# kan-bayashi/ParallelWaveGAN

Measured on AMD Instinct MI355X. Metric: HiFi-GAN V1 22.05 kHz generator inference RTF^-1 (audio samples/s), higher is better.
Workload: dtype f32; 1 GPU; HiFi-GAN V1 generator fwd, LJSpeech 22.05 kHz, B16 x 800 mel frames per GPU, fp32, random init; global_batch=16, parallelism=replicas x1

## Files before the change

### include/pwg_kernels.h

```cpp
#ifndef PWG_KERNELS_H_
#define PWG_KERNELS_H_

#include <stddef.h>
#include <stdint.h>

#ifdef __cplusplus
extern "C" {
#endif

typedef enum pwg_status {
  PWG_OK = 0,
  PWG_ERR_BAD_SHAPE = -1,
  PWG_ERR_UNSUPPORTED = -2,
  PWG_ERR_LAUNCH = -3,
  PWG_ERR_NULL = -4,
  PWG_ERR_WORKSPACE = -5
} pwg_status;

const char* pwg_last_error(void);
int pwg_abi_version(void);
int pwg_target_arch(void);

int pwg_prof_enable(int on);
int pwg_prof_reset(void);
// ... 64 lines not shown
int pwg_conv1d_backward_weight(const pwg_conv1d_desc* d, const float* x, const float* dy, float* dw,
                               float* db, float* workspace, size_t workspace_floats, void* stream);

size_t pwg_conv1d_backward_weight_wn_workspace_floats(const pwg_conv1d_desc* d);
int pwg_conv1d_backward_weight_wn(const pwg_conv1d_desc* d, const float* x, const float* dy, const float* v,
                                  const float* g, float* dv, float* dg, float* db, float* workspace,
                                  size_t workspace_floats, void* stream);

int pwg_conv1d_num_tile_configs(void);
int pwg_conv1d_forward_cfg(const pwg_conv1d_desc* d, const float* x, const float* w_packed,
                           const float* bias, const float* add1, const float* add2, float* y,
                           int32_t tile_config, int32_t use_dma, void* stream);

int pwg_conv1d_bf16_supported(const pwg_conv1d_desc* d);
size_t pwg_conv1d_bf16_packed_weight_bytes(const pwg_conv1d_desc* d);
int pwg_conv1d_bf16_pack_weight(const pwg_conv1d_desc* d, const float* w, const float* scale, void* w_packed,
                                void* stream);
int pwg_conv1d_bf16_forward(const pwg_conv1d_desc* d, const float* x, const void* w_packed, const float* bias,
                            const float* add1, const float* add2, float* y, float* workspace, size_t workspace_floats,
                            void* stream);
int pwg_conv1d_bf16_forward_cfg(const pwg_conv1d_desc* d, const float* x, const void* w_packed, const float* bias,
                                const float* add1, const float* add2, float* y, int32_t mfma_shape, void* stream);

int pwg_conv1d_split_supported(const pwg_conv1d_desc* d);
size_t pwg_conv1d_split_packed_weight_bytes(const pwg_conv1d_desc* d);
int pwg_conv1d_split_pack_weight(const pwg_conv1d_desc* d, const float* w, const float* scale, void* w_packed,
                                 void* stream);
int pwg_conv1d_split_forward(const pwg_conv1d_desc* d, const float* x, const void* w_packed, const float* bias,
                             const float* add1, const float* add2, float* y, float* workspace, size_t workspace_floats,
                             void* stream);
int pwg_conv1d_split_forward_cfg(const pwg_conv1d_desc* d, const float* x, const void* w_packed, const float* bias,
                                 const float* add1, const float* add2, float* y, int32_t mfma_shape, int32_t tile_mode,
                                 void* stream);

int pwg_conv1d_stream_supported(const pwg_conv1d_desc* d);
size_t pwg_conv1d_stream_hist_floats(const pwg_conv1d_desc* d);
int pwg_conv1d_stream_forward(const pwg_conv1d_desc* d, const float* x, const float* hist_in, float* hist_out,
                              const float* w_packed, const float* bias, const float* add1, const float* add2, float* y,
                              void* stream);

int pwg_conv1d_stream_bf16_supported(const pwg_conv1d_desc* d);
int pwg_conv1d_stream_bf16_forward(const pwg_conv1d_desc* d, const float* x, const float* hist_in, float* hist_out,
                                   const void* w_packed_bf16, const float* bias, const float* add1,
                                   const float* add2, float* y, void* stream);

int pwg_conv1d_stream_delayed_supported(const pwg_conv1d_desc* d, int32_t delay1, int32_t delay2);
int pwg_conv1d_stream_delayed_forward(const pwg_conv1d_desc* d, const float* x, const float* hist_in, float* hist_out,
                                      const float* w_packed, const float* bias, const float* add1,
                                      const float* add1_hist_in, float* add1_hist_out, int32_t delay1, const float* add2,
                                      const float* add2_hist_in, float* add2_hist_out, int32_t delay2, int32_t valid_lo,
                                      int32_t valid_hi, float* y, void* stream);

int pwg_conv1d_stream_bf16_delayed_supported(const pwg_conv1d_desc* d, int32_t delay1, int32_t delay2);
int pwg_conv1d_stream_bf16_delayed_forward(const pwg_conv1d_desc* d, const float* x, const float* hist_in,
                                           float* hist_out, const void* w_packed_bf16, const float* bias,
                                           const float* add1, const float* add1_hist_in, float* add1_hist_out,
                                           int32_t delay1, const float* add2, const float* add2_hist_in,
                                           float* add2_hist_out, int32_t delay2, int32_t valid_lo, int32_t valid_hi,
                                           float* y, void* stream);

int pwg_conv1d_stream_mirrored_supported(const pwg_conv1d_desc* d);
int pwg_conv1d_stream_mirrored_forward(const pwg_conv1d_desc* d, const float* x, const float* hist_in, float* hist_out,
                                       const float* w_packed, const float* bias, float* y, int32_t in_lo, int32_t in_hi,
                                       int32_t valid_lo, int32_t valid_hi, void* stream);

int pwg_conv1d_plan(const pwg_conv1d_desc* d, int32_t has_addends, int32_t* out);
// ... 310 lines not shown
```

### parallelwavegan_amd/_lib.py

```python
import ctypes
import os

_HERE = os.path.dirname(os.path.abspath(__file__))
LIB_PATH = os.environ.get("PWG_KERNEL_LIB") or os.path.join(_HERE, "libpwgkernels.so")

PWG_ACT_NONE, PWG_ACT_LEAKY_RELU, PWG_ACT_TANH, PWG_ACT_RELU = 0, 1, 2, 3
PWG_PAD_ZERO, PWG_PAD_REFLECT, PWG_PAD_REPLICATE = 0, 1, 2
ABI_VERSION = 15
SPECTRAL_NORM_SCRATCH_FLOATS = 257


class ConvDesc(ctypes.Structure):

    _fields_ = [
        ("batch", ctypes.c_int32),
        ("c_in", ctypes.c_int32),
        ("c_out", ctypes.c_int32),
        ("t_in", ctypes.c_int32),
        ("t_out", ctypes.c_int32),
        ("width", ctypes.c_int32),
        ("kernel", ctypes.c_int32),
        ("stride", ctypes.c_int32),
        ("dilation", ctypes.c_int32),
        ("pad_left", ctypes.c_int32),
# ... 76 lines not shown
_i64 = ctypes.c_int64
_f32 = ctypes.c_float

SIGNATURES = {
    "pwg_last_error": (ctypes.c_char_p, []),
    "pwg_abi_version": (ctypes.c_int, []),
    "pwg_target_arch": (ctypes.c_int, []),
    "pwg_debug_poison_lds": (ctypes.c_int, [ctypes.c_int]),
    "pwg_set_concurrency_hint": (ctypes.c_float, [ctypes.c_float]),
    "pwg_prof_enable": (ctypes.c_int, [ctypes.c_int]),
    "pwg_prof_reset": (ctypes.c_int, []),
    "pwg_prof_num_kernels": (ctypes.c_int, []),
    "pwg_prof_get": (ctypes.c_int, [_i32, ctypes.c_char_p, ctypes.c_size_t, ctypes.POINTER(ctypes.c_double),
                                    ctypes.POINTER(ctypes.c_int64), ctypes.POINTER(ctypes.c_double),
                                    ctypes.POINTER(ctypes.c_double)]),
    "pwg_conv1d_packed_weight_floats": (ctypes.c_size_t, [ctypes.POINTER(ConvDesc)]),
    "pwg_conv1d_pack_weight": (ctypes.c_int, [ctypes.POINTER(ConvDesc), _vp, _vp, _vp, _vp]),
    "pwg_conv1d_forward_workspace_floats": (ctypes.c_size_t, [ctypes.POINTER(ConvDesc)]),
    "pwg_conv1d_forward": (ctypes.c_int, [ctypes.POINTER(ConvDesc), _vp, _vp, _vp, _vp, _vp, _vp, _vp, ctypes.c_size_t,
                                          _vp]),
    "pwg_conv1d_bf16_supported": (ctypes.c_int, [ctypes.POINTER(ConvDesc)]),
    "pwg_conv1d_bf16_packed_weight_bytes": (ctypes.c_size_t, [ctypes.POINTER(ConvDesc)]),
    "pwg_conv1d_bf16_pack_weight": (ctypes.c_int, [ctypes.POINTER(ConvDesc), _vp, _vp, _vp, _vp]),
    "pwg_conv1d_bf16_forward": (ctypes.c_int, [ctypes.POINTER(ConvDesc), _vp, _vp, _vp, _vp, _vp, _vp, _vp, ctypes.c_size_t,
                                               _vp]),
    "pwg_conv1d_bf16_forward_cfg": (ctypes.c_int, [ctypes.POINTER(ConvDesc), _vp, _vp, _vp, _vp, _vp, _vp, _i32, _vp]),
    "pwg_conv1d_split_supported": (ctypes.c_int, [ctypes.POINTER(ConvDesc)]),
    "pwg_conv1d_split_packed_weight_bytes": (ctypes.c_size_t, [ctypes.POINTER(ConvDesc)]),
    "pwg_conv1d_split_pack_weight": (ctypes.c_int, [ctypes.POINTER(ConvDesc), _vp, _vp, _vp, _vp]),
    "pwg_conv1d_split_forward": (ctypes.c_int, [ctypes.POINTER(ConvDesc), _vp, _vp, _vp, _vp, _vp, _vp, _vp,
                                                ctypes.c_size_t, _vp]),
    "pwg_conv1d_split_forward_cfg": (ctypes.c_int, [ctypes.POINTER(ConvDesc), _vp, _vp, _vp, _vp, _vp, _vp, _i32, _i32,
                                                    _vp]),
    "pwg_conv1d_stream_supported": (ctypes.c_int, [ctypes.POINTER(ConvDesc)]),
    "pwg_conv1d_stream_hist_floats": (ctypes.c_size_t, [ctypes.POINTER(ConvDesc)]),
    "pwg_conv1d_stream_forward": (ctypes.c_int, [ctypes.POINTER(ConvDesc), _vp, _vp, _vp, _vp, _vp, _vp, _vp, _vp, _vp]),
    "pwg_conv1d_stream_bf16_supported": (ctypes.c_int, [ctypes.POINTER(ConvDesc)]),
    "pwg_conv1d_stream_bf16_forward": (ctypes.c_int, [ctypes.POINTER(ConvDesc), _vp, _vp, _vp, _vp, _vp, _vp, _vp, _vp,
                                                      _vp]),
    "pwg_conv1d_stream_delayed_supported": (ctypes.c_int, [ctypes.POINTER(ConvDesc), _i32, _i32]),
    "pwg_conv1d_stream_delayed_forward": (ctypes.c_int, [ctypes.POINTER(ConvDesc), _vp, _vp, _vp, _vp, _vp, _vp, _vp, _vp,
                                                         _i32, _vp, _vp, _vp, _i32, _i32, _i32, _vp, _vp]),
    "pwg_conv1d_stream_bf16_delayed_supported": (ctypes.c_int, [ctypes.POINTER(ConvDesc), _i32, _i32]),
    "pwg_conv1d_stream_bf16_delayed_forward": (ctypes.c_int, [ctypes.POINTER(ConvDesc), _vp, _vp, _vp, _vp, _vp, _vp, _vp,
                                                              _vp, _i32, _vp, _vp, _vp, _i32, _i32, _i32, _vp, _vp]),
    "pwg_conv1d_stream_mirrored_supported": (ctypes.c_int, [ctypes.POINTER(ConvDesc)]),
    "pwg_conv1d_stream_mirrored_forward": (ctypes.c_int, [ctypes.POINTER(ConvDesc), _vp, _vp, _vp, _vp, _vp, _vp, _i32,
                                                          _i32, _i32, _i32, _vp]),
    "pwg_conv1d_packed_weight_bwd_floats": (ctypes.c_size_t, [ctypes.POINTER(ConvDesc)]),
    "pwg_conv1d_pack_weight_bwd": (ctypes.c_int, [ctypes.POINTER(ConvDesc), _vp, _vp, _vp, _vp]),
    "pwg_weight_bank_table_bytes": (ctypes.c_size_t, [_i32]),
    "pwg_weight_bank_build": (ctypes.c_int, [ctypes.POINTER(BankItem), _i32, _vp, ctypes.c_size_t,
                                             ctypes.POINTER(ctypes.c_int32)]),
    "pwg_weight_bank_prepare": (ctypes.c_int, [_vp, ctypes.POINTER(ctypes.c_int32), _i32, _vp]),
    "pwg_conv1d_backward_data_workspace_floats": (ctypes.c_size_t, [ctypes.POINTER(ConvDesc)]),
    "pwg_conv1d_backward_data": (ctypes.c_int, [ctypes.POINTER(ConvDesc), _vp, _vp, _vp, _vp, _vp, _vp, ctypes.c_size_t,
                                                _vp]),
    "pwg_conv1d_backward_weight_workspace_floats": (ctypes.c_size_t, [ctypes.POINTER(ConvDesc)]),
    "pwg_conv1d_backward_weight": (ctypes.c_int, [ctypes.POINTER(ConvDesc), _vp, _vp, _vp, _vp, _vp, ctypes.c_size_t, _vp]),
    "pwg_conv1d_backward_weight_wn_workspace_floats": (ctypes.c_size_t, [ctypes.POINTER(ConvDesc)]),
    "pwg_conv1d_backward_weight_wn": (ctypes.c_int, [ctypes.POINTER(ConvDesc), _vp, _vp, _vp, _vp, _vp, _vp, _vp, _vp,
                                                     ctypes.c_size_t, _vp]),
    "pwg_conv1d_num_tile_configs": (ctypes.c_int, []),
    "pwg_conv1d_forward_cfg": (ctypes.c_int, [ctypes.POINTER(ConvDesc), _vp, _vp, _vp, _vp, _vp, _vp, _i32, _i32, _vp]),
    "pwg_conv1d_plan": (ctypes.c_int, [ctypes.POINTER(ConvDesc), _i32, ctypes.POINTER(_i32)]),
    "pwg_conv1d_backward_weight_plan": (ctypes.c_int, [ctypes.POINTER(ConvDesc), _i32, _i32, ctypes.POINTER(_i32)]),
# ... 147 lines not shown
```

### parallelwavegan_amd/csrc/conv1d_split.hip

```cpp
#include "mfma_conv.h"

namespace pwg {
namespace {

constexpr int PARTS = 3;

struct SplitArgs : MfmaConvArgs {
  int plane;
  long part_stride;
  float pre_mul;
  unsigned pre_mask;
  int wide_out;
};

static int split_geometry(const pwg_conv1d_desc* d, MfmaConvGeom* g) {
  return mfma_conv_geometry("conv1d_split", PARTS, false, d, g);
}

__device__ __forceinline__ float pre_activate(float v, float mul, unsigned mask) {
  const float n = __uint_as_float(__float_as_uint(v * mul) & mask);
  return v > 0.f ? v : n;
}

template <int NT, bool CHECKED>
// ... 186 lines not shown
    }
    __syncthreads();
    for (int tap = 0; tap < a.taps; ++tap) {
#pragma unroll
      for (int ks = 0; ks < KSTEPS; ++ks) {
        const int oct = ks * HL + c.h;
        const bf16x8* __restrict__ wp =
            image_rows(a.w, a.cin_chunks, a.m_pad, tap, chunk, oct) + c.m0 + c.wave_m * (WM * 32) + c.r;
        split_step<TILE, TM, TN, kConvRow, true>(wp, a.part_stride, xs, c.sh + c.wave_n * (WN * 32) + c.r + tap * a.dil,
                                                 oct * 8, a.plane, acc);
      }
    }
  }

  const size_t out_base = (size_t)c.b * a.c_out * a.t_out;
  const int row0 = c.m0 + c.wave_m * (WM * 32) + c.r, col0 = c.q0 + c.wave_n * (WN * 32) + 4 * c.h;
  const bool full = c.m0 + MT <= a.m && c.q0 + NT <= a.nq;
  if (!a.wide_out)
    split_epilogue<TILE, TM, TN, false, false>(a, acc, row0, col0, out_base);
  else if (full)
    split_epilogue<TILE, TM, TN, true, true>(a, acc, row0, col0, out_base);
  else
    split_epilogue<TILE, TM, TN, true, false>(a, acc, row0, col0, out_base);
}

template <bool VEC>
struct Family {
  template <int TILE, int WM, int WN, int WAVES_M>
  struct K {
    static constexpr auto fn = conv1d_split_mfma_kernel<TILE, WM, WN, WAVES_M, VEC>;
  };
};

static int split_forward(const pwg_conv1d_desc* d, const float* x, const void* w_packed, const float* bias,
                         const float* add1, const float* add2, float* y, int mfma_shape, int tile_mode,
                         hipStream_t stream) {
  MfmaConvGeom g;
  int rc = split_geometry(d, &g);
  if (rc == PWG_OK) rc = mfma_conv_check_forward("conv1d_split", d, x, w_packed, y, mfma_shape, tile_mode);
  if (rc != PWG_OK) return rc;
  const MfmaConvPlan p = mfma_conv_plan(d, g, PARTS, tile_mode, x, add1, add2);
  SplitArgs a;
  mfma_conv_fill_args(&a, d, g, x, w_packed, bias, add1, add2, y);
  a.plane = p.plane;
  a.part_stride = image_elems(g) / 8;
  a.pre_mul = d->pre_act == PWG_ACT_LEAKY_RELU ? d->pre_slope : (d->pre_act == PWG_ACT_RELU ? 0.0f : 1.0f);
  a.pre_mask = d->pre_act == PWG_ACT_RELU ? 0u : ~0u;
  a.wide_out = d->t_out % 4 == 0 && ((reinterpret_cast<uintptr_t>(y) | reinterpret_cast<uintptr_t>(add1) |
                                      reinterpret_cast<uintptr_t>(add2)) & 15u) == 0;
  maybe_poison_lds(stream);
  ProfScope prof(stream, "conv1d_split_mfma_kernel", p.flops, p.bytes);
  if (p.vec)
    mfma_conv_launch<Family<true>::K>(p, mfma_shape, a, stream);
  else
    mfma_conv_launch<Family<false>::K>(p, mfma_shape, a, stream);
  PWG_CHECK_LAUNCH("conv1d_split");
  return PWG_OK;
}

constexpr int kDefaultMfmaShape = 16;

}
}

using namespace pwg;

extern "C" int pwg_conv1d_split_supported(const pwg_conv1d_desc* d) {
  MfmaConvGeom g;
  return split_geometry(d, &g) == PWG_OK ? 1 : 0;
}

extern "C" size_t pwg_conv1d_split_packed_weight_bytes(const pwg_conv1d_desc* d) {
  MfmaConvGeom g;
  if (split_geometry(d, &g) != PWG_OK) return 0;
  return (size_t)PARTS * image_elems(g) * sizeof(__bf16);
}

extern "C" int pwg_conv1d_split_pack_weight(const pwg_conv1d_desc* d, const float* w, const float* scale, void* w_packed,
                                            void* stream) {
  MfmaConvGeom g;
  int rc = split_geometry(d, &g);
  if (rc != PWG_OK) return rc;
  PWG_REQUIRE(w && w_packed, PWG_ERR_NULL, "conv1d_split_pack_weight: NULL pointer");
  mfma_conv_pack<PARTS>(d, g, w, scale, w_packed, (hipStream_t)stream);
  PWG_CHECK_LAUNCH("conv1d_split_pack_weight");
  return PWG_OK;
}

extern "C" int pwg_conv1d_split_forward(const pwg_conv1d_desc* d, const float* x, const void* w_packed, const float* bias,
                                        const float* add1, const float* add2, float* y, float* workspace,
                                        size_t workspace_floats, void* stream) {
  (void)workspace;
  (void)workspace_floats;
  return split_forward(d, x, w_packed, bias, add1, add2, y, kDefaultMfmaShape, 0, (hipStream_t)stream);
}

extern "C" int pwg_conv1d_split_forward_cfg(const pwg_conv1d_desc* d, const float* x, const void* w_packed,
                                            const float* bias, const float* add1, const float* add2, float* y,
                                            int32_t mfma_shape, int32_t tile_mode, void* stream) {
  return split_forward(d, x, w_packed, bias, add1, add2, y, mfma_shape, tile_mode, (hipStream_t)stream);
}
```

### parallelwavegan_amd/functional.py

```python
import ctypes
import math
import os

import torch

from . import _lib, ops
from .ops import _ptr, _require_device, _stream

_L = _lib.lib


def _c(t):
    return t if t.is_contiguous() else t.contiguous()


class WeightNormFn(torch.autograd.Function):

    @staticmethod
    def forward(ctx, v, g):
        v = _c(v)
        g = _c(g)
        scale = ops.weight_norm_scale(v, g.reshape(-1))
        ctx.save_for_backward(v, g)
        return ops.scale_rows(v, scale)
# ... 29 lines not shown
class SpectralNormFn(torch.autograd.Function):

    @staticmethod
    def forward(ctx, w_orig, u, v, do_iter, eps):
        w_orig = _c(w_orig)
        _require_device(w_orig, u, v)
        rows = w_orig.shape[0]
        cols = w_orig.numel() // rows
        sigma = torch.empty(1, device=w_orig.device, dtype=torch.float32)
        w = torch.empty_like(w_orig)
        tmp = torch.empty(max(rows, 32 * cols), device=w_orig.device, dtype=torch.float32)
        u_saved, v_saved = (torch.empty_like(u), torch.empty_like(v)) if do_iter else (u.clone(), v.clone())
        _lib.check(_L().pwg_spectral_norm_forward_saved(_ptr(w_orig), _ptr(u), _ptr(v), _ptr(sigma), _ptr(w), _ptr(tmp),
                                                        _ptr(u_saved), _ptr(v_saved), rows, cols, int(bool(do_iter)),
                                                        float(eps), _stream()), "spectral_norm_forward_saved")
        ctx.save_for_backward(w_orig, u_saved, v_saved, sigma)
        return w

    @staticmethod
    def backward(ctx, dw):
        w_orig, u, v, sigma = ctx.saved_tensors
        dw = _c(dw)
        rows = w_orig.shape[0]
        cols = w_orig.numel() // rows
        dwo = torch.empty_like(w_orig)
        scratch = torch.empty(_lib.SPECTRAL_NORM_SCRATCH_FLOATS, device=dw.device, dtype=torch.float32)
        _lib.check(_L().pwg_spectral_norm_backward(_ptr(dw), _ptr(w_orig), _ptr(u), _ptr(v), _ptr(sigma), _ptr(dwo),
                                                   _ptr(scratch), rows, cols, _stream()), "spectral_norm_backward")
        return dwo, None, None, None, None


class PreparedWeights:

    __slots__ = ("key", "w", "_scale", "_fwd", "_fwd_desc", "_bwd", "_res", "_bf16", "_split", "_stale")

    def __init__(self, key, w, scale, fwd=None, fwd_desc=None, bwd=None):
        self.key, self.w, self._scale, self._fwd, self._fwd_desc, self._bwd, self._res = key, w, scale, fwd, fwd_desc, bwd, None
        self._bf16 = None
        self._split = None
        self._stale = False

    @property
    def scale(self):
        self._check()
        return self._scale

    def _check(self):
        if self._stale:
            raise RuntimeError("these prepared weights were overwritten by a later WeightBank.ensure(): a backward pass "
                               "through a graph built before the last parameter update is not supported with a "
                               "weight bank (call backward before the optimizer step, or disable the bank)")

    def _image(self, slot, pack, *desc):
        self._check()
        img = getattr(self, slot)
        if img is None:
            with torch.no_grad():
                img = pack(*desc, self.w, self._scale)
            setattr(self, slot, img)
        return img

    @property
    def fwd(self):
        return self._image("_fwd", ops.pack_weight, self._fwd_desc)

    def res(self):
        return self._image("_res", ops.resunit_pack_weight)

    def bf16(self):
        return self._image("_bf16", ops.pack_weight_bf16, self._fwd_desc)

    def split(self):
        return self._image("_split", ops.pack_weight_split, self._fwd_desc)

    def bwd(self, desc):
        return self._image("_bwd", ops.pack_weight_bwd, desc)


class FusedConvFn(torch.autograd.Function):

    @staticmethod
    def forward(ctx, x, w, bias, add1, add2, geom, fused, packed, g=None, precomputed=None):
        x = _c(x)
        b = x.shape[0]
        width = geom.get("width", 1)
        t_in = x.shape[-1] // width if x.dim() == 3 else x.shape[2]
        x3 = x.reshape(b, x.shape[1], -1)
        c_in = x3.shape[1]
        transposed = geom["transposed"]
        k = geom["kernel"]
        if transposed:
            c_out = w.shape[1] * geom["groups"]
            t_out = ops.conv_transpose_out_length(t_in, k, geom["stride"], geom["padding"], geom["output_padding"])
        else:
            c_out = w.shape[0]
            t_out = geom.get("t_out")
            if t_out is None:
                t_out = ops.conv_out_length(t_in, k, geom["stride"], geom["dilation"], geom["padding"],
                                            geom.get("padding_right", geom["padding"]))
        desc = ops.make_conv_desc(b, c_in, c_out, t_in, t_out, k, geom["stride"], geom["dilation"], geom["padding"],
                                  geom["groups"], transposed=transposed, width=width,
                                  pad_mode=geom.get("pad_mode", "zero"), **fused)
        wc = _c(w.reshape(w.shape[0], w.shape[1], -1))
        holder = packed if isinstance(packed, PreparedWeights) else None
        if holder is None:
            scale = None
# ... 870 lines not shown
```

### parallelwavegan_amd/layers/conv.py

```python
import math
import os

import torch

from .. import functional as Fn
from .. import ops


class _ConvNd(torch.nn.Module):
    transposed = False
    width_mode = False
    explicit_pad_min_elems = 1 << 20
    fold_batch = {"0": False, "1": True}.get(os.environ.get("PWG_FOLD_BATCH", ""), True)
    fold_max_cols = int(os.environ.get("PWG_FOLD_MAX_COLS", 40))
    fold_min_weight_bytes = 4 << 20
    precision = "fp32"
    split_exact = {"0": False, "1": True}.get(os.environ.get("PWG_SPLIT_EXACT", ""), True)
    split_admit_all = False

    def __init__(self, in_channels, out_channels, kernel_size, stride=1, padding=0, dilation=1, groups=1,
                 bias=True, output_padding=0, pad_mode="zero"):
        super().__init__()
        if in_channels % groups or out_channels % groups:
            raise ValueError("in_channels and out_channels must be divisible by groups")
# ... 133 lines not shown
            with torch.no_grad():
                if self.has_weight_norm:
                    v = self._w3(self.weight_v.detach())
                    scale = ops.weight_norm_scale(v, self.weight_g.detach().reshape(-1).contiguous())
                    self._cache_packed = Fn.PreparedWeights(key, v, scale, None, desc)
                else:
                    w = self._w3(self.effective_weight())
                    self._cache_packed = Fn.PreparedWeights(key, w, None, None, desc)
        return self._cache_packed

    def adopt_prepared(self, pw):
        self._cache_packed = pw

    def holds_current(self, pw):
        return self._cache_packed is pw and pw.key == self._params_key()

    def _packed(self, pack, cached):
        if self.has_spectral_norm and self.training:
            return pack(self.make_desc(1, self._probe_len()), self._w3(self.effective_weight()))
        return cached(self.prepared())

    def packed_weight(self):
        return self._packed(ops.pack_weight, lambda pw: pw.fwd)

    def packed_weight_bf16(self):
        return self._packed(ops.pack_weight_bf16, lambda pw: pw.bf16())

    def packed_weight_split(self):
        return self._packed(ops.pack_weight_split, lambda pw: pw.split())

    def _split_route(self, desc, needs_grad=False):
        return split_admitted(desc.c_in, desc.c_out, desc.kernel, desc.batch * desc.t_out, needs_grad,
                              self.split_exact, self.split_admit_all) and ops.conv1d_split_supported(desc)

    def bf16_capable(self):
        return not self.width_mode and ops.conv1d_bf16_supported(self.make_desc(1, self._probe_len()))

    @staticmethod
    def _w3(w):
        return w.reshape(w.shape[0], w.shape[1], -1).contiguous()

    def _probe_len(self):
        return self.kernel_size * self.dilation + self.stride + max(0, -self.padding_right)

    def geom(self):
        return dict(kernel=self.kernel_size, stride=self.stride, dilation=self.dilation, padding=self.padding,
                    padding_right=self.padding_right, groups=self.groups, transposed=self.transposed,
                    output_padding=self.output_padding, width=1, pad_mode=self.pad_mode)

    def out_length(self, t_in):
        raise NotImplementedError

    def make_desc(self, batch, t_in, width=1, **fused):
        raise NotImplementedError

    def _needs_grad(self, *tensors):
        if not torch.is_grad_enabled():
            return False
        if any(p.requires_grad for p in self.parameters(recurse=False)):
            return True
        return any(t is not None and t.requires_grad for t in tensors)

    def _fold_batch(self, x, add1, add2, precomputed):
        if not self.fold_batch or self.width_mode or self.transposed or x.dim() != 3 or self.pad_mode != "zero":
            return False
        if add1 is not None or add2 is not None or precomputed is not None:
# ... 28 lines not shown
                assert precomputed is None
                return Fn.FusedConvFn.apply(x, self.weight_tensor(), self.bias, add1, add2, geom, fused, None)
            if self.has_weight_norm:
                return Fn.FusedConvFn.apply(x, self.weight_v, self.bias, add1, add2, geom, fused, self.prepared(),
                                            self.weight_g, precomputed)
            return Fn.FusedConvFn.apply(x, self.weight, self.bias, add1, add2, geom, fused, self.prepared(), None,
                                        precomputed)
        assert precomputed is None, "precomputed outputs only make sense on the autograd path"
        with torch.no_grad():
            b = x.shape[0]
            if width_mode:
                h, width = x.shape[2], x.shape[3]
                desc = self.make_desc(b, h, width=width, **fused)
                y = ops.conv1d_forward(desc, x.reshape(b, x.shape[1], -1).contiguous(), self.packed_weight(),
                                       None if self.bias is None else self.bias.detach(),
                                       None if add1 is None else add1.reshape(b, self.out_channels, -1),
                                       None if add2 is None else add2.reshape(b, self.out_channels, -1))
                return y.reshape(b, self.out_channels, desc.t_out, width)
            if (self.pad_mode != "zero" and (self.padding > 0 or self.padding_right > 0) and not self.transposed
                    and x.numel() >= self.explicit_pad_min_elems):
                xp = Fn.pad1d(x, self.padding, self.padding_right, self.pad_mode)
                t_out = self.out_length(x.shape[-1])
                desc = ops.make_conv_desc(b, self.in_channels, self.out_channels, xp.shape[-1], t_out, self.kernel_size,
                                          self.stride, self.dilation, 0, self.groups, transposed=False, **fused)
                return ops.conv1d_forward(desc, xp, self.packed_weight(),
                                          None if self.bias is None else self.bias.detach(), add1, add2)
            desc = self.make_desc(b, x.shape[-1], **fused)
            if self.precision == "bf16" and ops.conv1d_bf16_supported(desc):
                return ops.conv1d_forward_bf16(desc, x.contiguous(), self.packed_weight_bf16(),
                                               None if self.bias is None else self.bias.detach(), add1, add2)
            if self.precision == "fp32" and self._split_route(desc):
                return ops.conv1d_forward_split(desc, x.contiguous(), self.packed_weight_split(),
                                                None if self.bias is None else self.bias.detach(), add1, add2)
            return ops.conv1d_forward(desc, x.contiguous(), self.packed_weight(),
                                      None if self.bias is None else self.bias.detach(), add1, add2)

    def extra_repr(self):
        norm = "weight_norm" if self.has_weight_norm else ("spectral_norm" if self.has_spectral_norm else "none")
        return (f"{self.in_channels}, {self.out_channels}, kernel_size={self.kernel_size}, stride={self.stride}, "
                f"padding={self.padding}, dilation={self.dilation}, groups={self.groups}, norm={norm}")


SPLIT_ADMITTED = {
    (128, 128, 7): 6400,
    (128, 128, 11): 6400,
    (256, 256, 7): 6400,
    (256, 256, 11): 6400,
}


def split_admitted(c_in, c_out, kernel, cols, needs_grad, enabled=True, admit_all=False):
    if needs_grad or not enabled:
        return False
    if admit_all:
        return True
    min_cols = SPLIT_ADMITTED.get((c_in, c_out, kernel))
    return min_cols is not None and cols >= min_cols


RESUNIT_SPLIT_MIN_COLS = 20480
RESUNIT_SPLIT_ADMITTED = {
    (64, 3, True): ("unit", 20480),
    (64, 7, True): ("pair", 20480),
    (64, 11, True): ("pair", 20480),
    (32, 7, True): ("unit", 25600),
    (32, 11, True): ("unit", 25600),
}


def resunit_split_admitted(channels, kernel, has_conv2, cols, needs_grad, enabled=True, admit_all=False):
    if needs_grad or not enabled:
        return None
    if admit_all:
        return "unit"
    form, min_cols = RESUNIT_SPLIT_ADMITTED.get((channels, kernel, bool(has_conv2)), (None, 0))
    return form if form is not None and cols >= max(min_cols, RESUNIT_SPLIT_MIN_COLS) else None


def each_conv(module):
    return (m for m in module.modules() if isinstance(m, _ConvNd))


def group_image(owner, slot, convs, pack, *extra):
    key = extra + tuple(cv._params_key() for cv in convs)
    held = getattr(owner, slot, None)
    if held is None or held[0] != key:
        hs = [cv.prepared() for cv in convs]
        with torch.no_grad():
            held = (key, pack(*(t for h in hs for t in (h.w, h.scale))))
        setattr(owner, slot, held)
# ... 59 lines not shown
```

### parallelwavegan_amd/ops.py

```python
import ctypes

import torch

from . import _lib
from ._lib import ConvDesc, ResUnitDesc, WaveNetDesc

ACT = {None: _lib.PWG_ACT_NONE, "none": _lib.PWG_ACT_NONE, "leaky_relu": _lib.PWG_ACT_LEAKY_RELU,
       "tanh": _lib.PWG_ACT_TANH, "relu": _lib.PWG_ACT_RELU}
PAD = {"zero": _lib.PWG_PAD_ZERO, "reflect": _lib.PWG_PAD_REFLECT, "replicate": _lib.PWG_PAD_REPLICATE}


PARAM_EPOCH = [0]


def bump_param_epoch():
    PARAM_EPOCH[0] += 1


def cache_epoch():
    return PARAM_EPOCH[0]


def param_epoch(p):
    return getattr(p, "_pwg_epoch", 0)
# ... 121 lines not shown
    return out


def _workspace(n_floats, device):
    if not n_floats:
        return None, 0
    return torch.empty(n_floats, device=device, dtype=torch.float32), n_floats


def conv1d_forward(desc, x, w_packed, bias=None, add1=None, add2=None, out=None):
    _require_device(x, w_packed, bias, add1, add2, out)
    if out is None:
        out = torch.empty((desc.batch, desc.c_out, desc.t_out * desc.width), device=x.device, dtype=torch.float32)
    assert x.numel() == desc.batch * desc.c_in * desc.t_in * desc.width, (tuple(x.shape), desc.batch, desc.c_in, desc.t_in)
    assert out.numel() == desc.batch * desc.c_out * desc.t_out * desc.width
    ws, ws_n = _workspace(_lib.lib().pwg_conv1d_forward_workspace_floats(ctypes.byref(desc)), x.device)
    _lib.check(_lib.lib().pwg_conv1d_forward(ctypes.byref(desc), _ptr(x), _ptr(w_packed), _ptr(bias), _ptr(add1),
                                             _ptr(add2), _ptr(out), _ptr(ws), ws_n, _stream()), "conv1d_forward")
    return out


def conv1d_bf16_supported(desc):
    return bool(_lib.lib().pwg_conv1d_bf16_supported(ctypes.byref(desc)))


def _zero_padded(desc):
    if desc.pad_mode == PAD["zero"]:
        return desc
    desc = ConvDesc.from_buffer_copy(desc)
    desc.pad_mode = PAD["zero"]
    return desc


def _pack_weight_mfma(kind, desc, w, scale):
    _require_device(w, scale)
    n = getattr(_lib.lib(), f"pwg_conv1d_{kind}_packed_weight_bytes")(ctypes.byref(desc))
    if n == 0:
        _lib.check(-1, f"conv1d_{kind}_packed_weight_bytes")
    out = torch.empty(n, device=w.device, dtype=torch.uint8)
    pack = getattr(_lib.lib(), f"pwg_conv1d_{kind}_pack_weight")
    _lib.check(pack(ctypes.byref(desc), _ptr(w), _ptr(scale), _ptr(out), _stream()), f"conv1d_{kind}_pack_weight")
    return out


def _conv1d_forward_mfma(kind, desc, image_desc, x, w_packed, bias, add1, add2, out, cfg):
    name = f"conv1d_forward_{kind}"
    _require_device(x, bias, add1, add2, out)
    if not w_packed.is_cuda or w_packed.dtype != torch.uint8:
        raise RuntimeError(f"{name}: w_packed must be the device image of pack_weight_{kind}")
    if out is None:
        out = torch.empty((desc.batch, desc.c_out, desc.t_out), device=x.device, dtype=torch.float32)
    assert x.numel() == desc.batch * desc.c_in * desc.t_in, (tuple(x.shape), desc.batch, desc.c_in, desc.t_in)
    assert out.numel() == desc.batch * desc.c_out * desc.t_out
    image_bytes = getattr(_lib.lib(), f"pwg_conv1d_{kind}_packed_weight_bytes")(ctypes.byref(image_desc))
    if image_bytes == 0:
        _lib.check(-1, f"conv1d_{kind}_packed_weight_bytes")
    assert w_packed.numel() == image_bytes, f"{name}: w_packed is not this layer's {kind} image"
    for t in (add1, add2):
        assert t is None or t.numel() == out.numel()
    args = (ctypes.byref(desc), _ptr(x), _ptr(w_packed), _ptr(bias), _ptr(add1), _ptr(add2), _ptr(out))
    if cfg is None:
        rc = getattr(_lib.lib(), f"pwg_conv1d_{kind}_forward")(*args, None, 0, _stream())
    else:
        rc = getattr(_lib.lib(), f"pwg_conv1d_{kind}_forward_cfg")(*args, *cfg, _stream())
    _lib.check(rc, name)
    return out


def pack_weight_bf16(desc, w, scale=None):
    return _pack_weight_mfma("bf16", _zero_padded(desc), w, scale)


def conv1d_forward_bf16(desc, x, w_packed, bias=None, add1=None, add2=None, out=None, mfma_shape=None):
    return _conv1d_forward_mfma("bf16", desc, _zero_padded(desc), x, w_packed, bias, add1, add2, out,
                                None if mfma_shape is None else (int(mfma_shape),))


def conv1d_split_supported(desc):
    return bool(_lib.lib().pwg_conv1d_split_supported(ctypes.byref(desc)))


def pack_weight_split(desc, w, scale=None):
    return _pack_weight_mfma("split", desc, w, scale)


def conv1d_forward_split(desc, x, w_packed, bias=None, add1=None, add2=None, out=None, mfma_shape=None, tile_mode=0):
    cfg = None if mfma_shape is None and not tile_mode else (int(mfma_shape or 16), int(tile_mode))
    return _conv1d_forward_mfma("split", desc, desc, x, w_packed, bias, add1, add2, out, cfg)


def conv1d_stream_supported(desc):
    return bool(_lib.lib().pwg_conv1d_stream_supported(ctypes.byref(desc)))


def conv1d_stream_hist_floats(desc):
    return _lib.lib().pwg_conv1d_stream_hist_floats(ctypes.byref(desc))


def _conv1d_stream_out(desc, x, hist_in, hist_out, add1, add2, out):
    if out is None:
        out = torch.empty((desc.batch, desc.c_out, desc.t_out), device=x.device, dtype=torch.float32)
    assert x.numel() == desc.batch * desc.c_in * desc.t_in, (tuple(x.shape), desc.batch, desc.c_in, desc.t_in)
    assert out.numel() == desc.batch * desc.c_out * desc.t_out
    n_hist = conv1d_stream_hist_floats(desc)
    for t in (hist_in, hist_out):
        assert t is None or t.numel() == n_hist, (tuple(t.shape), n_hist)
    for t in (add1, add2):
        assert t is None or t.numel() == out.numel()
    return out


def conv1d_stream_forward(desc, x, hist_in, hist_out, w_packed, bias=None, add1=None, add2=None, out=None):
    _require_device(x, hist_in, hist_out, w_packed, bias, add1, add2, out)
    out = _conv1d_stream_out(desc, x, hist_in, hist_out, add1, add2, out)
    _lib.check(_lib.lib().pwg_conv1d_stream_forward(ctypes.byref(desc), _ptr(x), _ptr(hist_in), _ptr(hist_out),
                                                    _ptr(w_packed), _ptr(bias), _ptr(add1), _ptr(add2), _ptr(out),
                                                    _stream()), "conv1d_stream_forward")
    return out


def conv1d_stream_delayed_supported(desc, delay1=0, delay2=0):
# ... 632 lines not shown
```

Before: 74.38 million samples/s.

## Route fp32 transposed-conv upsample layers through split-bf16 MFMA kernel

Adds a transposed-convolution variant of the split-bf16 MFMA conv kernel, using a phase-decomposed output mapping with a phase-aware epilogue for bias, residual adds and activation. The HiFi-GAN upsample layers (kernel = 2*stride) are admitted to this path via a per-shape minimum-column table. The aim is to replace the generic fp32 transposed conv with matrix-core execution while keeping fp32-level accuracy through the split representation. It adds substantial new kernel code with edge-handling paths that could have boundary bugs.

```diff
diff --git a/include/pwg_kernels.h b/include/pwg_kernels.h
--- a/include/pwg_kernels.h
+++ b/include/pwg_kernels.h
@@ -120,6 +120,17 @@
 int pwg_conv1d_split_forward_cfg(const pwg_conv1d_desc* d, const float* x, const void* w_packed, const float* bias,
                                  const float* add1, const float* add2, float* y, int32_t mfma_shape, int32_t tile_mode,
                                  void* stream);
+
+int pwg_convtr1d_split_supported(const pwg_conv1d_desc* d);
+size_t pwg_convtr1d_split_packed_weight_bytes(const pwg_conv1d_desc* d);
+int pwg_convtr1d_split_pack_weight(const pwg_conv1d_desc* d, const float* w, const float* scale, void* w_packed,
+                                   void* stream);
+int pwg_convtr1d_split_forward(const pwg_conv1d_desc* d, const float* x, const void* w_packed, const float* bias,
+                               const float* add1, const float* add2, float* y, float* workspace,
+                               size_t workspace_floats, void* stream);
+int pwg_convtr1d_split_forward_cfg(const pwg_conv1d_desc* d, const float* x, const void* w_packed, const float* bias,
+                                   const float* add1, const float* add2, float* y, int32_t mfma_shape,
+                                   int32_t tile_mode, void* stream);
 
 int pwg_conv1d_stream_supported(const pwg_conv1d_desc* d);
 size_t pwg_conv1d_stream_hist_floats(const pwg_conv1d_desc* d);
diff --git a/parallelwavegan_amd/_lib.py b/parallelwavegan_amd/_lib.py
--- a/parallelwavegan_amd/_lib.py
+++ b/parallelwavegan_amd/_lib.py
@@ -132,6 +132,13 @@
                                                 ctypes.c_size_t, _vp]),
     "pwg_conv1d_split_forward_cfg": (ctypes.c_int, [ctypes.POINTER(ConvDesc), _vp, _vp, _vp, _vp, _vp, _vp, _i32, _i32,
                                                     _vp]),
+    "pwg_convtr1d_split_supported": (ctypes.c_int, [ctypes.POINTER(ConvDesc)]),
+    "pwg_convtr1d_split_packed_weight_bytes": (ctypes.c_size_t, [ctypes.POINTER(ConvDesc)]),
+    "pwg_convtr1d_split_pack_weight": (ctypes.c_int, [ctypes.POINTER(ConvDesc), _vp, _vp, _vp, _vp]),
+    "pwg_convtr1d_split_forward": (ctypes.c_int, [ctypes.POINTER(ConvDesc), _vp, _vp, _vp, _vp, _vp, _vp, _vp,
+                                                  ctypes.c_size_t, _vp]),
+    "pwg_convtr1d_split_forward_cfg": (ctypes.c_int, [ctypes.POINTER(ConvDesc), _vp, _vp, _vp, _vp, _vp, _vp, _i32, _i32,
+                                                      _vp]),
     "pwg_conv1d_stream_supported": (ctypes.c_int, [ctypes.POINTER(ConvDesc)]),
     "pwg_conv1d_stream_hist_floats": (ctypes.c_size_t, [ctypes.POINTER(ConvDesc)]),
     "pwg_conv1d_stream_forward": (ctypes.c_int, [ctypes.POINTER(ConvDesc), _vp, _vp, _vp, _vp, _vp, _vp, _vp, _vp, _vp]),
diff --git a/parallelwavegan_amd/csrc/conv1d_split.hip b/parallelwavegan_amd/csrc/conv1d_split.hip
--- a/parallelwavegan_amd/csrc/conv1d_split.hip
+++ b/parallelwavegan_amd/csrc/conv1d_split.hip
@@ -242,6 +242,18 @@
   };
 };
 
+static void split_fill_args(SplitArgs* a, const pwg_conv1d_desc* d, const MfmaConvGeom& g, const MfmaConvPlan& p,
+                            const float* x, const void* w_packed, const float* bias, const float* add1, const float* add2,
+                            float* y) {
+  mfma_conv_fill_args(a, d, g, x, w_packed, bias, add1, add2, y);
+  a->plane = p.plane;
+  a->part_stride = image_elems(g) / 8;
+  a->pre_mul = d->pre_act == PWG_ACT_LEAKY_RELU ? d->pre_slope : (d->pre_act == PWG_ACT_RELU ? 0.0f : 1.0f);
+  a->pre_mask = d->pre_act == PWG_ACT_RELU ? 0u : ~0u;
+  a->wide_out = d->t_out % 4 == 0 && ((reinterpret_cast<uintptr_t>(y) | reinterpret_cast<uintptr_t>(add1) |
+                                       reinterpret_cast<uintptr_t>(add2)) & 15u) == 0;
+}
+
 static int split_forward(const pwg_conv1d_desc* d, const float* x, const void* w_packed, const float* bias,
                          const float* add1, const float* add2, float* y, int mfma_shape, int tile_mode,
                          hipStream_t stream) {
@@ -251,13 +263,7 @@
   if (rc != PWG_OK) return rc;
   const MfmaConvPlan p = mfma_conv_plan(d, g, PARTS, tile_mode, x, add1, add2);
   SplitArgs a;
-  mfma_conv_fill_args(&a, d, g, x, w_packed, bias, add1, add2, y);
-  a.plane = p.plane;
-  a.part_stride = image_elems(g) / 8;
-  a.pre_mul = d->pre_act == PWG_ACT_LEAKY_RELU ? d->pre_slope : (d->pre_act == PWG_ACT_RELU ? 0.0f : 1.0f);
-  a.pre_mask = d->pre_act == PWG_ACT_RELU ? 0u : ~0u;
-  a.wide_out = d->t_out % 4 == 0 && ((reinterpret_cast<uintptr_t>(y) | reinterpret_cast<uintptr_t>(add1) |
-                                      reinterpret_cast<uintptr_t>(add2)) & 15u) == 0;
+  split_fill_args(&a, d, g, p, x, w_packed, bias, add1, add2, y);
   maybe_poison_lds(stream);
   ProfScope prof(stream, "conv1d_split_mfma_kernel", p.flops, p.bytes);
   if (p.vec)
@@ -268,6 +274,255 @@
   return PWG_OK;
 }
 
+struct ConvtrArgs : SplitArgs {
+  int phases, out_off;
+};
+
+static int convtr_geometry(const pwg_conv1d_desc* d, MfmaConvGeom* g) {
+  PWG_REQUIRE(d != nullptr, PWG_ERR_NULL, "convtr1d_split: NULL descriptor");
+  PWG_REQUIRE(d->transposed, PWG_ERR_UNSUPPORTED,
+              "convtr1d_split: not a transposed convolution (a stride-1 Conv1d runs on conv1d_split)");
+  return mfma_conv_geometry("convtr1d_split", PARTS, true, d, g);
+}
+
+template <int NT, bool VEC>
+__device__ __forceinline__ void stage_chunk(const SplitArgs& a, const MfmaConvTile& c, int chunk, __bf16* xs) {
+  if (VEC) {
+    const int ngroups = (c.wcols + 3) >> 2, c_left = a.c_in - chunk * KC;
+    const float* __restrict__ xc = c.xb + (size_t)chunk * KC * a.t_in;
+    if (c.base >= 0 && c.base + 4 * ngroups <= a.t_in && c_left >= KC)
+      stage_window_vec<NT, false>(a, xc, c_left, c.base, ngroups, xs, c.tid);
+    else
+      stage_window_vec<NT, true>(a, xc, c_left, c.base, ngroups, xs, c.tid);
+  } else {
+    const int c_base = chunk * KC + c.wave * 8;
+    const bool interior = c.base >= 0 && c.base + c.wcols <= a.t_in && c_base + 8 <= a.c_in;
+    for (int col = c.lane; col < c.wcols; col += 64) {
+      const int t = c.base + col;
+      const float* __restrict__ src = c.xb + (size_t)c_base * a.t_in + t;
+      float f[8];
+      if (interior) {
+#pragma unroll
+        for (int j = 0; j < 8; ++j) f[j] = src[(size_t)j * a.t_in];
+      } else {
+        const bool tin = t >= 0 && t < a.t_in;
+#pragma unroll
+        for (int j = 0; j < 8; ++j) {
+          f[j] = 0.f;
+          if (tin && c_base + j < a.c_in) f[j] = src[(size_t)j * a.t_in];
+        }
+      }
+#pragma unroll
+      for (int j = 0; j < 8; ++j) f[j] = pre_activate(f[j], a.pre_mul, a.pre_mask);
+      split3_store<8>(f, xs + col * kConvRow + c.wave * 8, a.plane);
+    }
+  }
+}
+
+template <int N>
+__device__ __forceinline__ void convtr_finish(float out_mul, float out_div, int post_act, float post_slope, f32x4 (&v)[N],
+                                              const f32x4& bias, bool has_bias, bool has1, bool has2,
+                                              const f32x4 (&t1)[N], const f32x4 (&t2)[N]) {
+  if (has_bias) {
+#pragma unroll
+    for (int k = 0; k < N; ++k) v[k] += bias;
+  }
+  if (has1) {
+#pragma unroll
+    for (int k = 0; k < N; ++k) v[k] += t1[k];
+  }
+  if (has2) {
+#pragma unroll
+    for (int k = 0; k < N; ++k) v[k] += t2[k];
+  }
+  if (out_mul != 1.0f) {
+#pragma unroll
+    for (int k = 0; k < N; ++k) v[k] *= out_mul;
+  }
+  if (out_div != 1.0f) {
+#pragma unroll
+    for (int k = 0; k < N; ++k) v[k] = v[k] / out_div;
+  }
+  if (post_act == PWG_ACT_LEAKY_RELU) {
+#pragma unroll
+    for (int k = 0; k < N; ++k)
+#pragma unroll
+      for (int e = 0; e < 4; ++e) v[k][e] = v[k][e] > 0.f ? v[k][e] : v[k][e] * post_slope;
+  } else if (post_act == PWG_ACT_RELU) {
+#pragma unroll
+    for (int k = 0; k < N; ++k)
+#pragma unroll
+      for (int e = 0; e < 4; ++e) v[k][e] = v[k][e] > 0.f ? v[k][e] : 0.f;
+  } else if (post_act == PWG_ACT_TANH) {
+#pragma unroll
+    for (int k = 0; k < N; ++k) {
+#pragma unroll
+      for (int e = 0; e < 4; ++e) v[k][e] = tanhf(v[k][e]);
+      __builtin_amdgcn_sched_barrier(0);
+    }
+  }
+}
+
+template <int TILE, int TM, int TN, bool WIDE, bool FULL>
+__device__ __forceinline__ void convtr_epilogue(const ConvtrArgs& a, const typename Mfma<TILE>::acc_t (&acc)[TM][TN],
+                                                int row0, int col0, size_t out_base) {
+  constexpr int HL = 64 / TILE, NG = TILE * TILE / 64 / 4;
+  const bool has_bias = a.bias != nullptr, has1 = a.add1 != nullptr, has2 = a.add2 != nullptr;
+  const int s = a.phases, post_act = a.post_act;
+  const float out_mul = a.out_mul, out_div = a.out_div, post_slope = a.post_slope;
+#pragma unroll
+  for (int mi = 0; mi < TM; ++mi) {
+#pragma unroll
+    for (int g = 0; g < NG; ++g) {
+      const int m4 = row0 + mi * TILE + 4 * HL * g;
+      if (WIDE) {
+        const int mc = FULL ? m4 : min(m4, a.m - 4);
+        const int co = mc / s, ph = mc - co * s;
+        const size_t row = out_base + (size_t)co * a.t_out;
+        int o[TN];
+#pragma unroll
+        for (int ni = 0; ni < TN; ++ni) o[ni] = (col0 + ni * TILE) * s + ph - a.out_off;
+        auto load = [&](const float* __restrict__ src, f32x4 (&t)[TN]) {
+#pragma unroll
+          for (int ni = 0; ni < TN; ++ni)
+            t[ni] = *reinterpret_cast<const f32x4*>(src + row + (FULL ? o[ni] : min(max(o[ni], 0), a.t_out - 4)));
+        };
+        f32x4 t1[TN], t2[TN], v[TN];
+        float b = 0.f;
+        if (has_bias) b = a.bias[co];
+        if (has1) load(a.add1, t1);
+        if (has2) load(a.add2, t2);
+#pragma unroll
+        for (int ni = 0; ni < TN; ++ni)
+#pragma unroll
+          for (int e = 0; e < 4; ++e) v[ni][e] = acc[mi][ni][g * 4 + e];
+        const f32x4 bias = {b, b, b, b};
+        convtr_finish<TN>(out_mul, out_div, post_act, post_slope, v, bias, has_bias, has1, has2, t1, t2);
+#pragma unroll
+        for (int ni = 0; ni < TN; ++ni)
+          if (FULL || (m4 < a.m && o[ni] >= 0 && o[ni] < a.t_out)) *reinterpret_cast<f32x4*>(a.y + row + o[ni]) = v[ni];
+      } else {
+        int co = m4 / s, ph = m4 - co * s;
+        size_t row[4];
+        int phr[4];
+        f32x4 bias = {0.f, 0.f, 0.f, 0.f};
+#pragma unroll
+        for (int e = 0; e < 4; ++e) {
+          const int cc = min(co, a.c_out - 1);
+          row[e] = out_base + (size_t)cc * a.t_out;
+          phr[e] = ph - a.out_off;
+          if (has_bias) bias[e] = a.bias[cc];
+          if (++ph == s) ph = 0, ++co;
+        }
+#pragma unroll
+        for (int ni = 0; ni < TN; ++ni) {
+          const int qs = (col0 + ni * TILE) * s;
+          f32x4 t1[1], t2[1], v[1];
+          if (has1) {
+#pragma unroll
+            for (int e = 0; e < 4; ++e) t1[0][e] = a.add1[row[e] + min(max(qs + phr[e], 0), a.t_out - 1)];
+          }
+          if (has2) {
+#pragma unroll
+            for (int e = 0; e < 4; ++e) t2[0][e] = a.add2[row[e] + min(max(qs + phr[e], 0), a.t_out - 1)];
+          }
+#pragma unroll
+          for (int e = 0; e < 4; ++e) v[0][e] = acc[mi][ni][g * 4 + e];
+          convtr_finish<1>(out_mul, out_div, post_act, post_slope, v, bias, has_bias, has1, has2, t1, t2);
+#pragma unroll
+          for (int e = 0; e < 4; ++e) {
+            const int o = qs + phr[e];
+            if (m4 + e < a.m && o >= 0 && o < a.t_out) a.y[row[e] + o] = v[0][e];
+          }
+        }
+      }
+    }
+  }
+}
+
+template <int TILE, int WM, int WN, int WAVES_M, bool VEC>
+__global__ __launch_bounds__(256, WM * WN == 4 ? (TILE == 16 ? 3 : 2) : (WM * WN == 2 ? 3 : 4)) void
+convtr1d_split_mfma_kernel(ConvtrArgs a) {
+  constexpr int HL = 64 / TILE;
+  constexpr int KSTEPS = KC / (8 * HL);
+  constexpr int TM = WM * 32 / TILE, TN = WN * 32 / TILE;
+  constexpr int NREG = TILE * TILE / 64;
+  constexpr int WAVES_N = 4 / WAVES_M;
+  constexpr int MT = WAVES_M * WM * 32, NT = WAVES_N * WN * 32;
+  typedef typename Mfma<TILE>::acc_t acc_t;
+
+  extern __shared__ __attribute__((aligned(16))) unsigned char smem[];
+  __bf16* xs = reinterpret_cast<__bf16*>(smem);
+
+  const MfmaConvTile c = mfma_conv_tile<TILE, MT, NT, WAVES_M, VEC>(a);
+
+  acc_t acc[TM][TN];
+#pragma unroll
+  for (int mi = 0; mi < TM; ++mi)
+#pragma unroll
+    for (int ni = 0; ni < TN; ++ni)
+#pragma unroll
+      for (int i = 0; i < NREG; ++i) acc[mi][ni][i] = 0.f;
+
+  for (int chunk = 0; chunk < a.cin_chunks; ++chunk) {
+    if (chunk) __syncthreads();
+    stage_chunk<NT, VEC>(a, c, chunk, xs);
+    __syncthreads();
+    for (int tap = 0; tap < a.taps; ++tap) {
+#pragma unroll
+      for (int ks = 0; ks < KSTEPS; ++ks) {
+        const int oct = ks * HL + c.h;
+        const bf16x8* __restrict__ wp =
+            image_rows(a.w, a.cin_chunks, a.m_pad, tap, chunk, oct) + c.m0 + c.wave_m * (WM * 32) + c.r;
+        split_step<TILE, TM, TN, kConvRow, false>(wp, a.part_stride, xs, c.sh + c.wave_n * (WN * 32) + c.r + tap * a.dil,
+                                                  oct * 8, a.plane, acc);
+      }
+    }
+  }
+
+  const size_t out_base = (size_t)c.b * a.c_out * a.t_out;
+  const int row0 = c.m0 + c.wave_m * (WM * 32) + 4 * c.h, col0 = c.q0 + c.wave_n * (WN * 32) + c.r;
+  const bool full = c.m0 + MT <= a.m && c.q0 * a.phases >= a.out_off && (c.q0 + NT) * a.phases - a.out_off <= a.t_out;
+  if (!a.wide_out)
+    convtr_epilogue<TILE, TM, TN, false, false>(a, acc, row0, col0, out_base);
+  else if (full)
+    convtr_epilogue<TILE, TM, TN, true, true>(a, acc, row0, col0, out_base);
+  else
+    convtr_epilogue<TILE, TM, TN, true, false>(a, acc, row0, col0, out_base);
+}
+
+template <bool VEC>
+struct ConvtrFamily {
+  template <int TILE, int WM, int WN, int WAVES_M>
+  struct K {
+    static constexpr auto fn = convtr1d_split_mfma_kernel<TILE, WM, WN, WAVES_M, VEC>;
+  };
+};
+
+static int convtr_forward(const pwg_conv1d_desc* d, const float* x, const void* w_packed, const float* bias,
+                          const float* add1, const float* add2, float* y, int mfma_shape, int tile_mode,
+                          hipStream_t stream) {
+  MfmaConvGeom g;
+  int rc = convtr_geometry(d, &g);
+  if (rc == PWG_OK) rc = mfma_conv_check_forward("convtr1d_split", d, x, w_packed, y, mfma_shape, tile_mode);
+  if (rc != PWG_OK) return rc;
+  PWG_REQUIRE((long)(g.nq + 256) * g.phases < (1L << 31), PWG_ERR_UNSUPPORTED, "convtr1d_split: output row too long");
+  const MfmaConvPlan p = mfma_conv_plan(d, g, PARTS, tile_mode, x, add1, add2);
+  ConvtrArgs a;
+  split_fill_args(&a, d, g, p, x, w_packed, bias, add1, add2, y);
+  a.phases = g.phases;
+  a.out_off = g.out_off;
+  a.wide_out = a.wide_out && g.phases % 4 == 0 && g.out_off % 4 == 0;
+  maybe_poison_lds(stream);
+  ProfScope prof(stream, "convtr1d_split_mfma_kernel", p.flops, p.bytes);
+  if (p.vec)
+    mfma_conv_launch<ConvtrFamily<true>::K>(p, mfma_shape, a, stream);
+  else
+    mfma_conv_launch<ConvtrFamily<false>::K>(p, mfma_shape, a, stream);
+  PWG_CHECK_LAUNCH("convtr1d_split");
+  return PWG_OK;
+}
+
 constexpr int kDefaultMfmaShape = 16;
 
 }
@@ -310,3 +565,39 @@
                                             int32_t mfma_shape, int32_t tile_mode, void* stream) {
   return split_forward(d, x, w_packed, bias, add1, add2, y, mfma_shape, tile_mode, (hipStream_t)stream);
 }
+
+extern "C" int pwg_convtr1d_split_supported(const pwg_conv1d_desc* d) {
+  MfmaConvGeom g;
+  return convtr_geometry(d, &g) == PWG_OK ? 1 : 0;
+}
+
+extern "C" size_t pwg_convtr1d_split_packed_weight_bytes(const pwg_conv1d_desc* d) {
+  MfmaConvGeom g;
+  if (convtr_geometry(d, &g) != PWG_OK) return 0;
+  return (size_t)PARTS * image_elems(g) * sizeof(__bf16);
+}
+
+extern "C" int pwg_convtr1d_split_pack_weight(const pwg_conv1d_desc* d, const float* w, const float* scale, void* w_packed,
+                                              void* stream) {
+  MfmaConvGeom g;
+  int rc = convtr_geometry(d, &g);
+  if (rc != PWG_OK) return rc;
+  PWG_REQUIRE(w && w_packed, PWG_ERR_NULL, "convtr1d_split_pack_weight: NULL pointer");
+  mfma_conv_pack<PARTS>(d, g, w, scale, w_packed, (hipStream_t)stream);
+  PWG_CHECK_LAUNCH("convtr1d_split_pack_weight");
+  return PWG_OK;
+}
+
+extern "C" int pwg_convtr1d_split_forward(const pwg_conv1d_desc* d, const float* x, const void* w_packed, const float* bias,
+                                          const float* add1, const float* add2, float* y, float* workspace,
+                                          size_t workspace_floats, void* stream) {
+  (void)workspace;
+  (void)workspace_floats;
+  return convtr_forward(d, x, w_packed, bias, add1, add2, y, kDefaultMfmaShape, 0, (hipStream_t)stream);
+}
+
+extern "C" int pwg_convtr1d_split_forward_cfg(const pwg_conv1d_desc* d, const float* x, const void* w_packed,
+                                              const float* bias, const float* add1, const float* add2, float* y,
+                                              int32_t mfma_shape, int32_t tile_mode, void* stream) {
+  return convtr_forward(d, x, w_packed, bias, add1, add2, y, mfma_shape, tile_mode, (hipStream_t)stream);
+}
diff --git a/parallelwavegan_amd/functional.py b/parallelwavegan_amd/functional.py
--- a/parallelwavegan_amd/functional.py
+++ b/parallelwavegan_amd/functional.py
@@ -85,12 +85,13 @@
 
 class PreparedWeights:
 
-    __slots__ = ("key", "w", "_scale", "_fwd", "_fwd_desc", "_bwd", "_res", "_bf16", "_split", "_stale")
+    __slots__ = ("key", "w", "_scale", "_fwd", "_fwd_desc", "_bwd", "_res", "_bf16", "_split", "_split_tr", "_stale")
 
     def __init__(self, key, w, scale, fwd=None, fwd_desc=None, bwd=None):
         self.key, self.w, self._scale, self._fwd, self._fwd_desc, self._bwd, self._res = key, w, scale, fwd, fwd_desc, bwd, None
         self._bf16 = None
         self._split = None
+        self._split_tr = None
         self._stale = False
 
     @property
@@ -125,6 +126,9 @@
 
     def split(self):
         return self._image("_split", ops.pack_weight_split, self._fwd_desc)
+
+    def split_transposed(self):
+        return self._image("_split_tr", ops.pack_weight_split_transposed, self._fwd_desc)
 
     def bwd(self, desc):
         return self._image("_bwd", ops.pack_weight_bwd, desc)
diff --git a/parallelwavegan_amd/layers/conv.py b/parallelwavegan_amd/layers/conv.py
--- a/parallelwavegan_amd/layers/conv.py
+++ b/parallelwavegan_amd/layers/conv.py
@@ -189,6 +189,15 @@
     def _split_route(self, desc, needs_grad=False):
         return split_admitted(desc.c_in, desc.c_out, desc.kernel, desc.batch * desc.t_out, needs_grad,
                               self.split_exact, self.split_admit_all) and ops.conv1d_split_supported(desc)
+
+    def packed_weight_split_transposed(self):
+        return self._packed(ops.pack_weight_split_transposed, lambda pw: pw.split_transposed())
+
+    def _upsample_split_route(self, desc, needs_grad=False):
+        return (self.transposed
+                and upsample_split_admitted(desc.c_in, desc.c_out, desc.kernel, desc.stride, desc.batch * desc.t_out,
+                                            needs_grad, self.split_exact, self.split_admit_all)
+                and ops.convtr1d_split_supported(desc))
 
     def bf16_capable(self):
         return not self.width_mode and ops.conv1d_bf16_supported(self.make_desc(1, self._probe_len()))
@@ -283,6 +292,9 @@
             if self.precision == "fp32" and self._split_route(desc):
                 return ops.conv1d_forward_split(desc, x.contiguous(), self.packed_weight_split(),
                                                 None if self.bias is None else self.bias.detach(), add1, add2)
+            if self.precision == "fp32" and self._upsample_split_route(desc):
+                return ops.conv1d_forward_split_transposed(desc, x.contiguous(), self.packed_weight_split_transposed(),
+                                                           None if self.bias is None else self.bias.detach(), add1, add2)
             return ops.conv1d_forward(desc, x.contiguous(), self.packed_weight(),
                                       None if self.bias is None else self.bias.detach(), add1, add2)
 
@@ -307,6 +319,24 @@
         return True
     min_cols = SPLIT_ADMITTED.get((c_in, c_out, kernel))
     return min_cols is not None and cols >= min_cols
+
+
+UPSAMPLE_SPLIT_MIN_COLS = 800
+UPSAMPLE_SPLIT_ADMITTED = {
+    (512, 256, 8): 102400,
+    (256, 128, 8): 6400,
+    (128, 64, 2): 12800,
+    (64, 32, 2): 25600,
+}
+
+
+def upsample_split_admitted(c_in, c_out, kernel, stride, cols, needs_grad, enabled=True, admit_all=False):
+    if needs_grad or not enabled or kernel != 2 * stride:
+        return False
+    if admit_all:
+        return True
+    min_cols = UPSAMPLE_SPLIT_ADMITTED.get((c_in, c_out, stride))
+    return min_cols is not None and cols >= max(min_cols, UPSAMPLE_SPLIT_MIN_COLS)
 
 
 RESUNIT_SPLIT_MIN_COLS = 20480
diff --git a/parallelwavegan_amd/ops.py b/parallelwavegan_amd/ops.py
--- a/parallelwavegan_amd/ops.py
+++ b/parallelwavegan_amd/ops.py
@@ -177,19 +177,19 @@
     return desc
 
 
-def _pack_weight_mfma(kind, desc, w, scale):
+def _pack_weight_mfma(kind, desc, w, scale, op="conv1d"):
     _require_device(w, scale)
-    n = getattr(_lib.lib(), f"pwg_conv1d_{kind}_packed_weight_bytes")(ctypes.byref(desc))
+    n = getattr(_lib.lib(), f"pwg_{op}_{kind}_packed_weight_bytes")(ctypes.byref(desc))
     if n == 0:
-        _lib.check(-1, f"conv1d_{kind}_packed_weight_bytes")
+        _lib.check(-1, f"{op}_{kind}_packed_weight_bytes")
     out = torch.empty(n, device=w.device, dtype=torch.uint8)
-    pack = getattr(_lib.lib(), f"pwg_conv1d_{kind}_pack_weight")
-    _lib.check(pack(ctypes.byref(desc), _ptr(w), _ptr(scale), _ptr(out), _stream()), f"conv1d_{kind}_pack_weight")
-    return out
-
-
-def _conv1d_forward_mfma(kind, desc, image_desc, x, w_packed, bias, add1, add2, out, cfg):
-    name = f"conv1d_forward_{kind}"
+    pack = getattr(_lib.lib(), f"pwg_{op}_{kind}_pack_weight")
+    _lib.check(pack(ctypes.byref(desc), _ptr(w), _ptr(scale), _ptr(out), _stream()), f"{op}_{kind}_pack_weight")
+    return out
+
+
+def _conv1d_forward_mfma(kind, desc, image_desc, x, w_packed, bias, add1, add2, out, cfg, op="conv1d"):
+    name = f"{op}_forward_{kind}"
     _require_device(x, bias, add1, add2, out)
     if not w_packed.is_cuda or w_packed.dtype != torch.uint8:
         raise RuntimeError(f"{name}: w_packed must be the device image of pack_weight_{kind}")
@@ -197,17 +197,17 @@
         out = torch.empty((desc.batch, desc.c_out, desc.t_out), device=x.device, dtype=torch.float32)
     assert x.numel() == desc.batch * desc.c_in * desc.t_in, (tuple(x.shape), desc.batch, desc.c_in, desc.t_in)
     assert out.numel() == desc.batch * desc.c_out * desc.t_out
-    image_bytes = getattr(_lib.lib(), f"pwg_conv1d_{kind}_packed_weight_bytes")(ctypes.byref(image_desc))
+    image_bytes = getattr(_lib.lib(), f"pwg_{op}_{kind}_packed_weight_bytes")(ctypes.byref(image_desc))
     if image_bytes == 0:
-        _lib.check(-1, f"conv1d_{kind}_packed_weight_bytes")
+        _lib.check(-1, f"{op}_{kind}_packed_weight_bytes")
     assert w_packed.numel() == image_bytes, f"{name}: w_packed is not this layer's {kind} image"
     for t in (add1, add2):
         assert t is None or t.numel() == out.numel()
     args = (ctypes.byref(desc), _ptr(x), _ptr(w_packed), _ptr(bias), _ptr(add1), _ptr(add2), _ptr(out))
     if cfg is None:
-        rc = getattr(_lib.lib(), f"pwg_conv1d_{kind}_forward")(*args, None, 0, _stream())
+        rc = getattr(_lib.lib(), f"pwg_{op}_{kind}_forward")(*args, None, 0, _stream())
     else:
-        rc = getattr(_lib.lib(), f"pwg_conv1d_{kind}_forward_cfg")(*args, *cfg, _stream())
+        rc = getattr(_lib.lib(), f"pwg_{op}_{kind}_forward_cfg")(*args, *cfg, _stream())
     _lib.check(rc, name)
     return out
 
@@ -232,6 +232,20 @@
 def conv1d_forward_split(desc, x, w_packed, bias=None, add1=None, add2=None, out=None, mfma_shape=None, tile_mode=0):
     cfg = None if mfma_shape is None and not tile_mode else (int(mfma_shape or 16), int(tile_mode))
     return _conv1d_forward_mfma("split", desc, desc, x, w_packed, bias, add1, add2, out, cfg)
+
+
+def convtr1d_split_supported(desc):
+    return bool(_lib.lib().pwg_convtr1d_split_supported(ctypes.byref(desc)))
+
+
+def pack_weight_split_transposed(desc, w, scale=None):
+    return _pack_weight_mfma("split", desc, w, scale, op="convtr1d")
+
+
+def conv1d_forward_split_transposed(desc, x, w_packed, bias=None, add1=None, add2=None, out=None, mfma_shape=None,
+                                    tile_mode=0):
+    cfg = None if mfma_shape is None and not tile_mode else (int(mfma_shape or 16), int(tile_mode))
+    return _conv1d_forward_mfma("split", desc, desc, x, w_packed, bias, add1, add2, out, cfg, op="convtr1d")
 
 
 def conv1d_stream_supported(desc):
```

Result: faster. 76.87 million samples/s, median of 6 (+3.4%).
